# Image-Processing-Systems-Laboratory/DeepInPainting

Measured on AMD Instinct MI355X. Metric: train images/sec at 256x256, batch 8/GPU, 1/2/4/8 MI355X; IPSR layer ms, higher is better.
Workload: dtype f32; 1 GPU; BASELINE config 2: 256x256 synthetic images, 128x128 centre mask (M=256 of N=1024 feature positions), batch 8/GPU, fp32, full IPSR training step; global_batch=8, parallelism=dp1, dropout=True, conv_math=fp32, vgg16=seeded random init (no pretrained weights offline)

## Files before the change

deepinpainting_amd/_lib.py:

```python
import ctypes
import os

_HERE = os.path.dirname(os.path.abspath(__file__))
LIB_PATH = os.path.join(_HERE, "libipsr_hip.so")
ABI_VERSION = 15

_lib = None

c_void_p, c_int, c_float, c_size_t = ctypes.c_void_p, ctypes.c_int, ctypes.c_float, ctypes.c_size_t

SIGNATURES = {
    "ipsr_abi_version": (c_int, []),
    "ipsr_last_error": (ctypes.c_char_p, []),
    "ipsr_feat_mask_workspace_bytes": (c_size_t, [c_int, c_int, c_int]),
    "ipsr_feat_mask": (c_int, [c_void_p, c_int, c_int, c_int, c_float, c_void_p, c_void_p, c_size_t, c_void_p]),
    "ipsr_index_prep": (c_int, [c_void_p, c_int, c_int, c_int, c_int, c_int, c_void_p, c_void_p, c_void_p, c_void_p]),
    "ipsr_patch_normalize": (c_int, [c_void_p, c_int, c_int, c_int, c_void_p, c_void_p, c_void_p]),
    "ipsr_corr_argmax_workspace_bytes": (c_size_t, [c_int, c_int, c_int]),
    "ipsr_corr_argmax": (c_int, [c_void_p, c_void_p, c_int, c_int, c_int, c_void_p, c_void_p, c_void_p,
                                 c_void_p, c_size_t, c_void_p]),
    "ipsr_bwd_index_ints": (c_size_t, [c_int, c_int]),
    "ipsr_forward_workspace_bytes": (c_size_t, [c_int] * 7),
    "ipsr_forward": (c_int, [c_void_p, c_void_p, c_void_p, c_int, c_int, c_int, c_int, c_int, c_int, c_int,
                             c_void_p, c_void_p, c_void_p, c_void_p, c_void_p, c_void_p, c_size_t, c_void_p]),
# ... 65 lines not shown
    "ipsr_l1_pair_loss_workspace_bytes": (c_size_t, [c_int]),
    "ipsr_l1_pair_loss": (c_int, [c_void_p, c_void_p, c_void_p, c_int, c_float, c_void_p, c_void_p, c_void_p, c_void_p, c_size_t, c_void_p]),
    "ipsr_loss_grad_scale": (c_int, [c_void_p, c_void_p, c_void_p, c_int, c_void_p, c_void_p, c_int, c_void_p]),
    "ipsr_profile_enable": (c_int, [c_int]),
    "ipsr_profile_enable_mask": (c_int, [c_int, ctypes.c_uint]),
    "ipsr_profile_read": (c_int, [c_void_p, c_int]),
    "ipsr_profile_read_region": (c_int, [c_int, c_void_p, c_int]),
    "ipsr_profile_read_region_work": (c_int, [c_int, c_void_p, c_void_p, c_int]),
    "ipsr_profile_read_region_work2": (c_int, [c_int, c_void_p, c_void_p, c_void_p, c_int]),
    "ipsr_conv3x3_winograd_mp": (c_int, [c_int, c_void_p, c_void_p, c_void_p, c_int, c_void_p, c_int, c_void_p, c_int, c_int, c_int, c_int, c_int, c_int, c_int,
                                         c_void_p, c_size_t, c_void_p]),
    "ipsr_conv3x3_winograd_wrw_mp": (c_int, [c_int, c_void_p, c_void_p, c_void_p, c_int, c_int, c_int, c_int, c_int, c_int, c_int, c_void_p, c_size_t, c_void_p]),
    "ipsr_conv4x4_winograd_mp": (c_int, [c_int, c_int, c_void_p, c_void_p, c_void_p, c_int, c_int, c_int, c_int, c_int, c_int, c_int, c_void_p, c_size_t, c_void_p]),
    "ipsr_conv4x4s2_winograd_mp": (c_int, [c_int, c_void_p, c_void_p, c_void_p, c_int, c_int, c_int, c_int, c_int, c_int, c_int, c_void_p, c_size_t, c_void_p]),
    "ipsr_conv3x3_bf16_workspace_bytes": (c_size_t, [c_int] * 6),
    "ipsr_conv3x3_bf16x3_workspace_bytes": (c_size_t, [c_int] * 6),
    "ipsr_conv3x3_bf16": (c_int, [c_int, c_void_p, c_void_p, c_void_p, c_int, c_int, c_int, c_int, c_int, c_int, c_void_p, c_size_t, c_void_p]),
    "ipsr_conv3x3_bf16_packed": (c_int, [c_int, c_void_p, c_void_p, c_void_p, c_int, c_int, c_int, c_int, c_int, c_int, c_int, c_void_p, c_size_t, c_void_p]),
    "ipsr_conv4x4s2_bf16_workspace_bytes": (c_size_t, [c_int] * 6),
    "ipsr_conv4x4s2_bf16": (c_int, [c_int, c_void_p, c_void_p, c_void_p, c_int, c_int, c_int, c_int, c_int, c_int, c_void_p, c_size_t, c_void_p]),
    "ipsr_conv4x4s2_bf16_dil_workspace_bytes": (c_size_t, [c_int] * 6),
    "ipsr_conv4x4s2_bf16_dil": (c_int, [c_int, c_void_p, c_void_p, c_void_p, c_int, c_int, c_int, c_int, c_int, c_int, c_void_p, c_size_t, c_void_p]),
    "ipsr_conv4x4s2_bf16x3_workspace_bytes": (c_size_t, [c_int] * 6),
    "ipsr_conv4x4s2_bf16x3": (c_int, [c_int, c_void_p, c_void_p, c_void_p, c_int, c_int, c_int, c_int, c_int, c_void_p, c_size_t, c_void_p]),
    "ipsr_conv4x4s2_bf16_wrw_workspace_bytes": (c_size_t, [c_int] * 5),
    "ipsr_conv4x4s2_bf16_wrw": (c_int, [c_void_p, c_void_p, c_void_p, c_int, c_int, c_int, c_int, c_int, c_void_p, c_size_t, c_void_p]),
    "ipsr_conv4x4s2_bf16x3_wrw_workspace_bytes": (c_size_t, [c_int] * 5),
    "ipsr_conv4x4s2_bf16x3_wrw": (c_int, [c_void_p, c_void_p, c_void_p, c_int, c_int, c_int, c_int, c_int, c_void_p, c_size_t, c_void_p]),
    "ipsr_conv3x3_bf16_wrw_workspace_bytes": (c_size_t, [c_int] * 6),
    "ipsr_conv4x4s2_bf16x3_dil_wrw_workspace_bytes": (c_size_t, [c_int] * 5),
    "ipsr_conv4x4s2_bf16x3_dil_wrw": (c_int, [c_void_p, c_void_p, c_void_p, c_int, c_int, c_int, c_int, c_int, c_void_p, c_size_t, c_void_p]),
    "ipsr_conv3x3_bf16x3_wrw_workspace_bytes": (c_size_t, [c_int] * 6),
    "ipsr_conv3x3_bf16_wrw": (c_int, [c_int, c_void_p, c_void_p, c_void_p, c_int, c_int, c_int, c_int, c_int, c_void_p, c_size_t, c_void_p]),
    "ipsr_wino_gemm_split": (c_int, [c_int, c_int, c_int, c_void_p]),
    "ipsr_debug_force_wino_split": (c_int, [c_int, c_int, c_int]),
    "ipsr_debug_set_option": (c_int, [c_int, c_int]),
}


class IpsrLibraryError(RuntimeError):
    pass


def lib():
    global _lib
    if _lib is not None:
        return _lib
    if not os.path.exists(LIB_PATH):
        raise IpsrLibraryError(
            "libipsr_hip.so not found at %s — build it with `python -c 'import __graft_entry__ as g; g.build()'` "
            "or `make -C deepinpainting_amd/csrc`.  The IPSR layer has no CPU/eager fallback." % LIB_PATH)
    import torch
    h = ctypes.CDLL(LIB_PATH)
    for name, (res, args) in SIGNATURES.items():
        fn = getattr(h, name)
        fn.restype = res
        fn.argtypes = args
    if h.ipsr_abi_version() != ABI_VERSION:
        raise IpsrLibraryError("libipsr_hip.so ABI %d != expected %d — rebuild" % (h.ipsr_abi_version(), ABI_VERSION))
    _lib = h
    return _lib


def check(rc, what):
    if rc == 0:
        return
# ... 5 lines not shown
```

deepinpainting_amd/models/IPSR.py:

```python
import os
from collections import OrderedDict

import torch

from . import networks
from .base_model import BaseModel
from .vgg16 import Vgg16
from .. import dist as ipsr_dist


class IPSR(BaseModel):
    def name(self):
        return 'IPSRModel'

    def initialize(self, opt):
        BaseModel.initialize(self, opt)
        self.opt = opt
        self.isTrain = opt.isTrain
        self.strict_reference = bool(getattr(opt, 'strict_reference', False))
        self.batch_vgg = bool(getattr(opt, 'batch_vgg', False))
        self.batch_disc = bool(getattr(opt, 'batch_disc', True))
        self.amp_bf16 = bool(getattr(opt, 'amp_bf16', False))
        from . import hipconv
        hipconv.set_conv_math(fp32=getattr(opt, 'conv_math', 'fp32'), bf16=getattr(opt, 'conv_math_bf16', 'bf16x3'))
# ... 12 lines not shown
                "seeded-random VGG16 instead.")
        self.vgg = Vgg16(requires_grad=False, weights_path=weights).to(self.device)
        self.vgg.eval()
        if not self.vgg.pretrained and not getattr(opt, 'quiet', False):
            print('WARNING: VGG16 feature extractor is seeded-random (allow_random_vgg) — not the pretrained net the reference uses')

        fs = opt.fineSize
        self.input_A = self.Tensor(opt.batchSize, opt.input_nc, fs, fs)
        self.input_B = self.Tensor(opt.batchSize, opt.output_nc, fs, fs)
        self.input_ref = self.Tensor(opt.batchSize, opt.output_nc, fs, fs)

        self.mask_global = torch.zeros(1, 1, fs, fs, dtype=torch.bool, device=self.device)
        lo, hi = int(fs / 4) + opt.overlap, int(fs / 2) + int(fs / 4) - opt.overlap
        self.mask_global[:, :, lo:hi, lo:hi] = 1
        self.mask_type = opt.mask_type
        self.gMask_opts = {}
        self.use_gpu = len(opt.gpu_ids) > 0

        self.netG, self.Cosis_list, self.Cosis_list2, self.CSA_model = networks.define_G(
            opt.input_nc_g, opt.output_nc, opt.ngf, opt.which_model_netG, opt, self.mask_global, opt.norm,
            opt.use_dropout, opt.init_type, self.gpu_ids, opt.init_gain)
        self.netP, _, _, _ = networks.define_G(
            opt.input_nc, opt.output_nc, opt.ngf, opt.which_model_netP, opt, self.mask_global, opt.norm,
            opt.use_dropout, opt.init_type, self.gpu_ids, opt.init_gain)
        self.CSA_model[0].corr_bf16 = self.amp_bf16 and bool(getattr(opt, 'bf16_corr', True)) and self.device.type == 'cuda'
        if self.isTrain:
            use_sigmoid = opt.gan_type == 'vanilla'
            self.netD = networks.define_D(opt.input_nc, opt.ndf, opt.which_model_netD, opt.n_layers_D, opt.norm,
                                          use_sigmoid, opt.init_type, self.gpu_ids, opt.init_gain)
            self.netF = networks.define_D(opt.input_nc, opt.ndf, opt.which_model_netF, opt.n_layers_D, opt.norm,
                                          use_sigmoid, opt.init_type, self.gpu_ids, opt.init_gain)

        reach = 0 if self.amp_bf16 else int(getattr(opt, 'smallmap_reach', 1024))
        for net in (self.netG, self.netP) + ((self.netD, self.netF) if self.isTrain else ()):
            for mod in net.modules():
                if isinstance(mod, (torch.nn.Conv2d, torch.nn.ConvTranspose2d)):
                    mod.smallmap_reach = reach or None

        if not self.isTrain or opt.continue_train:
            print('Loading pre-trained network!')
            self.load_network(self.netG, 'G', opt.which_epoch)
            self.load_network(self.netP, 'P', opt.which_epoch)
            if self.isTrain:
                self.load_network(self.netD, 'D', opt.which_epoch)
                self.load_network(self.netF, 'F', opt.which_epoch)

        self.criterionGAN = networks.GANLoss(gan_type=opt.gan_type)
        self.criterionL1 = torch.nn.L1Loss()
        self._gt_latent = None
        self._reducer_D = self._reducer_G = None

        if self.isTrain:
            self.old_lr = opt.lr
            fused = bool(getattr(opt, 'fused_adam', True)) and self.device.type == 'cuda'

            def mk(net):
                kw = dict(lr=opt.lr, betas=(opt.beta1, 0.999))
                if fused:
                    try:
                        return torch.optim.Adam(net.parameters(), fused=True, **kw)
                    except (TypeError, RuntimeError):
                        pass
                return torch.optim.Adam(net.parameters(), **kw)
            self.optimizer_G, self.optimizer_P = mk(self.netG), mk(self.netP)
            self.optimizer_D, self.optimizer_F = mk(self.netD), mk(self.netF)
            self.optimizers = [self.optimizer_G, self.optimizer_P, self.optimizer_D, self.optimizer_F]
            self.schedulers = [networks.get_scheduler(o, opt) for o in self.optimizers]

            if torch.distributed.is_available() and torch.distributed.is_initialized() \
                    and torch.distributed.get_world_size() > 1:
# ... 218 lines not shown
```

deepinpainting_amd/models/hipconv.py:

```python
import os
from collections import namedtuple

import torch
import torch.nn as nn
import torch.nn.functional as F

from .. import _lib, ops
from .. import dist as ipsr_dist

_FORCE = None
_MATH = {"fp32": "fp32", "bf16": "bf16x3"}


def set_conv_math(fp32=None, bf16=None):
    from .. import ops as _ops
    for key, val in (("fp32", fp32), ("bf16", bf16)):
        if val is not None:
            if val not in _ops.MATH_CODE or (key == "bf16" and val in _ops.DIRECT_PASSES):
                raise ValueError("conv math must be one of %s" % sorted(k for k in _ops.MATH_CODE if k))
            _MATH[key] = val
    _SEL.clear()


_DIRECT_DILATED = False
# ... 261 lines not shown
    if not (k == 3 and stride == 1 and pad == 1 and dil == 1) or H * W < 4096 or not engine_takes("thin", "data", op, lay, bf16):
        return False
    fwd = op in (ops.CONV_FWD, ops.CONVT_FWD)
    i, o = (Cin, Cout) if fwd else (Cout, Cin)
    if bf16:
        return i == 3
    return o in (3, 6) or i == 3


def _smallmap_op(op):
    return ops.SM_FWD if op in (ops.CONV_FWD, ops.CONVT_BWD_DATA) else ops.SM_DATA


def _smallmap_data_wins(op, lay):
    transposed, B, Cin, H, W, Cout, k, stride, pad, dil = lay
    if _env("IPSR_NO_SMALLMAP", "0") == "1" or k not in (3, 4) or min(Cin, Cout) < 256:
        return False
    g = _smallmap_geometry(lay)
    return g[3] >= 1 and g[4] >= 1 and g[0] * g[3] * g[4] <= int(_env("IPSR_SMALLMAP_MAX_POS", "32")) and engine_takes("smallmap", "data", op, lay, False)


def _smallmap_wrw_wins(lay):
    transposed, B, Cin, H, W, Cout, k, stride, pad, dil = lay
    if k != 4 or stride != 2 or _env("IPSR_NO_SMALLMAP", "0") == "1":
        return False
    g = _smallmap_geometry(lay)
    return g[3] >= 1 and g[4] >= 1 and g[0] * g[3] * g[4] <= 256 and min(Cin, Cout) >= 256 and engine_takes("smallmap", "wrw", None, lay, False)


def _is_k4s1(k, stride, pad, dil):
    return k == 4 and stride == 1 and pad == 1 and dil == 1


def select_wrw(transposed, B, Cin, H, W, Cout, k, stride, pad, dil, bf16=False, reach=None):
    key = (1, _FORCE, transposed, B, Cin, H, W, Cout, k, stride, pad, dil, bf16)
    eng = _SEL.get(key)
    if eng is None:
        eng = _SEL[key] = _select_wrw_any((transposed, B, Cin, H, W, Cout, k, stride, pad, dil), bf16)
    return _reached("wrw", key, eng, None, bf16, reach) if reach else eng


def _select_wrw_any(lay, bf16):
    transposed, B, Cin, H, W, Cout, k, stride, pad, dil = lay
    eng = _select_wrw(lay)
    thin = _mode() == "auto" and _env("IPSR_NO_THIN", "0") != "1" and pad == 1 and dil == 1 and (k, stride) in ((3, 1), (4, 2)) and H * W >= 4096 \
        and engine_takes("thin_mfma", "wrw", None, lay, bf16)
    if not bf16:
        eng = "thin_mfma" if thin and eng == "miopen" else _direct_opt_in("wrw", eng, None, lay)
    elif not (_bf16_wins(eng, Cin, H, W, Cout, True) or _ENGINES[eng].fp32_copies):
        eng = "thin_mfma" if thin else _bf16_direct_wrw(lay)
    return eng if engine_takes(eng, "wrw", None, lay, bf16) else "miopen"


def _bf16_direct_wrw(lay):
    transposed, B, Cin, H, W, Cout, k, stride, pad, dil = lay
    if _env("IPSR_BF16_ENGINES", "") == "none" or _mode() in ("miopen", "winograd", "direct"):
        return "miopen"
    if k == 3 and stride == 1 and pad == 1 and dil == 1 and H * W >= 1024 and engine_takes("bf16d", "wrw", None, lay, True):
        return "bf16d"
    g = _s2_geometry(lay)
    if g is not None and g[3] >= 32 and ((g[0] + 127) // 128) * ((g[1] + 31) // 32) >= 4 and engine_takes("bf16d", "wrw", None, lay, True):
        return "bf16d"
    return "miopen"


def _dil_geometry(lay):
    transposed, B, Cin, H, W, Cout, k, stride, pad, dil = lay
    if transposed or not _is_dilated4(k, stride, pad, dil) or H % 2 or W % 2:
        return None
    return Cout, Cin, H // 2, W // 2


# ... 32 lines not shown
def _select_wrw(lay):
    transposed, B, Cin, H, W, Cout, k, stride, pad, dil = lay
    mode = _mode()
    if mode == "auto" and not transposed and Cout == 1 and Cin >= 64 and engine_takes("one", "wrw", None, lay, False):
        return "one"
    if mode == "auto" and not transposed and _is_dilated4(k, stride, pad, dil) and min(Cin, Cout) >= 128 and 32 <= H <= 128 \
            and H % 2 == 0 and W % 2 == 0:
        return "wino_dil"
    if mode == "auto" and not transposed and _is_k4s1(k, stride, pad, dil) and min(Cin, Cout) >= 128 and 16 <= H <= 128 and W >= 4:
        return "wino_dil"
    if mode == "auto":
        g = _s2_geometry(lay)
        if g is not None and _s2_wins(g):
            return "wino_s2"
    if mode == "auto" and _smallmap_wrw_wins(lay):
        return "smallmap"
    ok = k == 3 and stride == 1 and pad == 1 and dil == 1
    if mode in ("miopen", "direct") or not ok:
        return "miopen"
    if mode == "winograd":
        return "winograd"
    if 256 <= H * W <= 4096 and max(Cin, Cout) >= 256 and min(Cin, Cout) >= 128:
        return "winograd"
    if transposed and Cout == 64 and Cin >= 256 and H * W <= 16384:
        return "winograd"
    return "miopen"


_Engine = namedtuple("_Engine", "data wrw takes bf16_io fp32_copies sink wrw_x_as_dy", defaults=(None, None, None, False, False, False, False))
_K3 = (3, 1, 1, 1)


def engine_takes(eng, kind, op, lay, bf16):
    return eng == "miopen" or bool(_ENGINES[eng].takes(kind, op, lay, bf16))


def _frozen_pack(w, param):
    param = w if param is None else param
    return dict(keep_packed=isinstance(param, nn.Parameter) and not param.requires_grad and not torch.is_grad_enabled(), pack_key=param)


def _fine_coarse(x, dy, lay):
    return ((dy, x) if lay[0] else (x, dy)) + (lay[1],) + _s2_geometry(lay)


def _direct_case(lay, x3):
    if lay[6:] == _K3:
        return "k3", None
    dilated = (x3 or _DIRECT_DILATED_BF16) and _is_dilated4(*lay[6:])
    g = _dil_geometry(lay) if dilated else _s2_geometry(lay)
    return (None if g is None else "dil" if dilated else "s2"), g


def _direct_mode(case, op):
    return _dil_mode(op) if case == "dil" else _s2_mode(op)


def _bf16d_data(op, inp, w, lay, math, out_dtype, param):
    if inp.dtype != torch.bfloat16:
        inp = inp.to(torch.bfloat16)
    case, g = _direct_case(lay, False)
    if case == "k3":
        return ops.conv3x3_bf16(op, inp, w, lay[1:5], lay[5], out_dtype=out_dtype, **_frozen_pack(w, param))
    if case == "dil":
        return ops.conv4x4s2_bf16_dil(_dil_mode(op) & ~ops.S2_DILATED, inp, w, lay[1], *g, out_dtype=out_dtype)
    return ops.conv4x4s2_bf16(_s2_mode(op), inp, w, lay[1], *g, out_dtype=out_dtype)

# ... 90 lines not shown
        lambda op, inp, w, lay, math, out_dtype, param: ops.conv4x4s2_winograd(_s2_mode(op), inp, w, lay[1], *_s2_geometry(lay), math=math, out_dtype=out_dtype),
        lambda x, dy, lay, math, sink: ops.conv4x4s2_winograd(ops.S2_WEIGHT_GRAD, *_fine_coarse(x, dy, lay), out=sink, math=math),
        _wino_s2_takes, bf16_io=True, sink=True, wrw_x_as_dy=True),
    "thin": _Engine(
        lambda op, inp, w, lay, math, out_dtype, param: ops.conv3x3_thin(op, inp, w, lay[1:5], lay[5], out_dtype=out_dtype),
        takes=lambda kind, op, lay, bf16: kind == "data" and lay[6:] == _K3 and ops.thin_supported(op, *lay[2:6])),
    "thin_f2m": _Engine(
        lambda op, inp, w, lay, math, out_dtype, param: ops.conv_thin_f2m_mfma(op, inp, w, lay[1:5], lay[5], lay[6], lay[7], out_dtype=out_dtype),
        takes=lambda kind, op, lay, bf16: kind == "data" and lay[8:] == (1, 1) and ops.thin_f2m_mfma_supported(op, *lay[1:8])),
    "thin_mfma": _Engine(
        None, _thin_mfma_wrw, sink=True,
        takes=lambda kind, op, lay, bf16: kind == "wrw" and lay[8:] == (1, 1) and ops.thin_wrw_mfma_supported(*lay[:8])),
    "smallmap": _Engine(
        lambda op, inp, w, lay, math, out_dtype, param, tiled=False: ops.conv_smallmap(_smallmap_op(op), inp, w, *_smallmap_geometry(lay), tiled=tiled),
        lambda x, dy, lay, math, sink, tiled=False: ops.conv_smallmap(ops.SM_WRW, *((x, dy) if lay[0] else (dy, x)), *_smallmap_geometry(lay), out=sink,
                                                                       tiled=tiled),
        lambda kind, op, lay, bf16, tiled=False: ops.smallmap_supported(_smallmap_op(op) if kind == "data" else ops.SM_WRW, *_smallmap_geometry(lay),
                                                                         tiled=tiled),
        fp32_copies=True, sink=True),
    "direct": _Engine(
        lambda op, inp, w, lay, math, out_dtype, param: ops.conv2d(op, inp, w, lay[1:5], *lay[5:]),
        takes=lambda kind, op, lay, bf16: kind == "data" and ops.conv2d_supported(op, *lay[1:])),
    "one": _Engine(
        lambda op, inp, w, lay, math, out_dtype, param: ops.conv_to_one(inp, w, lay[8]),
        lambda x, dy, lay, math, sink: ops.conv_to_one_wrw(x, dy, lay[6], lay[8], out=sink),
        lambda kind, op, lay, bf16: not lay[0] and lay[5] == 1 and (kind == "wrw" or op == ops.CONV_FWD) and ops.conv_to_one_supported(*lay[1:5], *lay[6:]),
        fp32_copies=True, sink=True),
    "bf16d": _Engine(_bf16d_data, _bf16d_wrw, _bf16d_takes, bf16_io=True, sink=True, wrw_x_as_dy=True),
    "bf16x3d": _Engine(_bf16x3d_data, takes=_bf16x3d_takes),
    "bf16x3w": _Engine(None, _bf16x3w_wrw, _bf16x3w_takes, sink=True),
    "miopen": _Engine(),
}


def _run_data(eng, op, inp, w, lay, math, out_dtype, param=None, tiled=False):
    e = _ENGINES[eng]
    kw = {"tiled": True} if tiled else {}
    if e.fp32_copies:
        return e.data(op, inp.float(), w, lay, math, torch.float32, param, **kw).to(out_dtype)
    return e.data(op, inp, w, lay, math, out_dtype, param, **kw)


def _run_wrw(eng, x, dy, w, lay, math, tiled=False):
    e = _ENGINES[eng]
    sink = ipsr_dist.grad_sink_for(w.data_ptr(), w.shape) if e.sink else None
    if e.fp32_copies:
        x, dy = x.float(), dy.float()
    elif e.wrw_x_as_dy and x.dtype != dy.dtype:
        x = x.to(dy.dtype)
    return e.wrw(x, dy, lay, math, sink, **({"tiled": True} if tiled else {}))


def _miopen_forward(x, w, transposed, stride, pad, dil):
    if x.dtype != w.dtype and not torch.is_autocast_enabled():
        w = w.to(x.dtype)
    return F.conv_transpose2d(x, w, None, stride, pad, 0, 1, dil) if transposed else F.conv2d(x, w, None, stride, pad, dil)


def _miopen_backward(dy, x, w, transposed, stride, pad, dil, which):
    dt = dy.dtype
    out = torch.ops.aten.convolution_backward(dy, x if x.dtype == dt else x.to(dt), w if w.dtype == dt else w.to(dt), None, [stride, stride],
                                              [pad, pad], [dil, dil], transposed, [0, 0], 1, which)
    return out[0], (out[1].to(w.dtype) if out[1] is not None else None)


class _HipConv(torch.autograd.Function):

    @staticmethod
    def forward(ctx, x, w, lay, eng_fwd, math, act, reach=None):
        transposed, B, Cin, H, W, Cout, k, stride, pad, dil = lay
        xc = x.contiguous()
        if eng_fwd == "miopen":
            y = _miopen_forward(xc, w, transposed, stride, pad, dil)
        else:
            fop = ops.CONVT_FWD if transposed else ops.CONV_FWD
            y = _run_data(eng_fwd, fop, xc, w, lay, math, act, tiled=eng_fwd == "smallmap" and _via_reach("data", fop, lay, act == torch.bfloat16, reach))
        ctx.save_for_backward(xc, w)
        ctx.lay, ctx.geom = lay, (transposed, k, stride, pad, dil, Cout)
        ctx.math, ctx.bf16, ctx.reach = math, act == torch.bfloat16, reach
        if _check_hook is not None:
            _check_hook("forward", eng_fwd, ctx.geom, (xc, w), y)
        return y

    @staticmethod
    def backward(ctx, dy):
        x, w = ctx.saved_tensors
        lay, math, bf16, reach = ctx.lay, ctx.math, ctx.bf16, ctx.reach
        transposed, B, Cin, H, W, Cout, k, stride, pad, dil = lay
        dy = dy.contiguous()
        if bf16 and dy.dtype != torch.bfloat16:
            dy = dy.to(torch.bfloat16)
        dx = dw = None
        if ctx.needs_input_grad[0]:
            op = ops.CONVT_BWD_DATA if transposed else ops.CONV_BWD_DATA
            eng = select(op, B, Cin, H, W, Cout, k, stride, pad, dil, bf16, reach=reach)
            if eng == "miopen":
                dx = _miopen_backward(dy, x, w, transposed, stride, pad, dil, [True, False, False])[0]
                if dx.dtype != x.dtype:
                    dx = dx.to(x.dtype)
            else:
                dx = _run_data(eng, op, dy, w, lay, math, x.dtype, tiled=eng == "smallmap" and _via_reach("data", op, lay, bf16, reach))
            if _check_hook is not None:
                _check_hook("input_grad", eng, ctx.geom, (dy, x, w), dx)
        if ctx.needs_input_grad[1]:
            weng = select_wrw(transposed, B, Cin, H, W, Cout, k, stride, pad, dil, bf16, reach=reach)
            if weng == "miopen":
                dw = _miopen_backward(dy, x, w, transposed, stride, pad, dil, [False, True, False])[1]
            else:
                dw = _run_wrw(weng, x, dy, w, lay, math, tiled=weng == "smallmap" and _via_reach("wrw", None, lay, bf16, reach))
            if _check_hook is not None:
                _check_hook("weight_grad", weng, ctx.geom, (dy, x, w), dw)
        return dx, dw, None, None, None, None, None


def _geometry(m):
    ks, st, pd, dl = m.kernel_size, m.stride, m.padding, m.dilation
    if m.groups != 1 or ks[0] != ks[1] or st[0] != st[1] or pd[0] != pd[1] or dl[0] != dl[1] or isinstance(pd, str):
        return None
    if isinstance(m, nn.ConvTranspose2d) and tuple(m.output_padding) != (0, 0):
        return None
    if getattr(m, "padding_mode", "zeros") != "zeros":
        return None
    return ks[0], st[0], pd[0], dl[0]


def _layer_of(m, x, w):
    g = _geometry(m)
    if g is None or not x.is_cuda or x.dim() != 4 or w.dtype != torch.float32 or x.dtype not in (torch.float32, torch.bfloat16):
        return None
    amp = _amp_bf16()
    if not amp and torch.is_autocast_enabled():
        return None
    transposed = isinstance(m, nn.ConvTranspose2d)
    B, Cin, H, W = x.shape
    return (transposed, B, Cin, H, W, w.shape[1] if transposed else w.shape[0]) + g, amp or x.dtype == torch.bfloat16


def conv_math(bf16):
    return _MATH["bf16" if bf16 else "fp32"]


def _engines_of(lay, bf16, dx=True, dw=True, reach=None):
    transposed, B, Cin, H, W, Cout, k, stride, pad, dil = lay
    fop, bop = (ops.CONVT_FWD, ops.CONVT_BWD_DATA) if transposed else (ops.CONV_FWD, ops.CONV_BWD_DATA)
    return (select(fop, B, Cin, H, W, Cout, k, stride, pad, dil, bf16, reach=reach),
            select(bop, B, Cin, H, W, Cout, k, stride, pad, dil, bf16, reach=reach) if dx else "miopen",
            select_wrw(transposed, B, Cin, H, W, Cout, k, stride, pad, dil, bf16, reach=reach) if dw else "miopen")


def any_engine(m, x):
    lb = _layer_of(m, x, m.weight)
    if lb is None:
        return False
    return _engines_of(*lb, reach=getattr(m, "smallmap_reach", None)) != ("miopen",) * 3


def conv_nobias(m, x, weight=None):
    w = m.weight if weight is None else weight
    lb = _layer_of(m, x, w)
    if lb is not None:
        lay, bf16 = lb
        act = torch.bfloat16 if bf16 else torch.float32
        math = _MATH["bf16" if bf16 else "fp32"]
        grad = torch.is_grad_enabled()
        reach = getattr(m, "smallmap_reach", None)
        engs = _engines_of(lay, bf16, grad and x.requires_grad, grad and w.requires_grad, reach)
        if grad and (x.requires_grad or w.requires_grad):
            if engs != ("miopen",) * 3:
                return _HipConv.apply(x, w, lay, engs[0], math, act, reach)
        elif engs[0] != "miopen":
            fop = ops.CONVT_FWD if lay[0] else ops.CONV_FWD
            return _run_data(engs[0], fop, x.contiguous(), w.detach(), lay, math, act, param=w,
                             tiled=engs[0] == "smallmap" and _via_reach("data", fop, lay, bf16, reach))
    if isinstance(m, nn.ConvTranspose2d):
        return F.conv_transpose2d(x, w, None, m.stride, m.padding, m.output_padding, m.groups, m.dilation)
    return F.conv2d(x, w, None, m.stride, m.padding, m.dilation, m.groups)
```

deepinpainting_amd/ops.py:

```python
import contextlib
import threading
import weakref
from collections import namedtuple

import torch

from . import _lib

_ws_cache = {}


def _stream():
    return torch._C._cuda_getCurrentRawStream(torch._C._cuda_getDevice())


def _workspace(nbytes, device):
    key = (device.index, _stream())
    buf = _ws_cache.get(key)
    if buf is None or buf.numel() < nbytes:
        buf = torch.empty(max(int(nbytes), 1 << 20), dtype=torch.uint8, device=device)
        _ws_cache[key] = buf
    return buf


# ... 847 lines not shown
               "ipsr_conv_thin_f2m_mfma")
    return out


def thin_wrw_mfma_supported(transposed, B, Cin, H, W, Cout, k, stride):
    if transposed:
        Kb, Cs, Hb, Wb = Cin, Cout, H, W
    else:
        if H % stride or W % stride:
            return False
        Kb, Cs, Hb, Wb = Cout, Cin, H // stride, W // stride
    return _lib.lib().ipsr_conv_thin_wrw_mfma_workspace_bytes(B, Kb, Cs, Hb, Wb, k, stride) > 0


def conv_thin_wrw_mfma(transposed, x, dy, k, stride, out=None):
    x, _ = _act(x, "x")
    dy, _ = _act(dy, "dy")
    big, small = (x, dy) if transposed else (dy, x)
    if big.dtype == torch.float32 and small.dtype != torch.float32:
        raise TypeError("conv_thin_wrw_mfma: an fp32 wide tensor needs an fp32 narrow one")
    B, Kb, Hb, Wb = big.shape
    Cs = small.shape[1]
    if tuple(small.shape) != (B, Cs, Hb * stride, Wb * stride):
        raise RuntimeError("conv_thin_wrw_mfma: narrow tensor %s does not match wide %s at stride %d" % (tuple(small.shape), tuple(big.shape), stride))
    L = _lib.lib()
    g = _result(out, (Kb, Cs, k, k), torch.float32, x.device, "conv_thin_wrw_mfma")
    ws = _probed_workspace(L, L.ipsr_conv_thin_wrw_mfma_workspace_bytes(B, Kb, Cs, Hb, Wb, k, stride), x.device,
                           "ipsr_conv_thin_wrw_mfma: Kb=%d Cs=%d %dx%d k%d s%d", (Kb, Cs, Hb, Wb, k, stride))
    _lib.check(L.ipsr_conv_thin_wrw_mfma(big.data_ptr(), small.data_ptr(), g.data_ptr(), B, Kb, Cs, Hb, Wb, k, stride, int(big.dtype == torch.bfloat16) | (2 if small.dtype == torch.bfloat16 else 0),
                                         ws.data_ptr(), ws.numel(), _stream()), "ipsr_conv_thin_wrw_mfma")
    return g


SM_DATA, SM_WRW, SM_FWD = 0, 1, 2


SM_TILED = 16


def smallmap_supported(op, B, R, Cq, Ho, Wo, Hf, Wf, k, stride, pad, dil, tiled=False):
    return _lib.lib().ipsr_conv_smallmap_workspace_bytes(op | (SM_TILED if tiled else 0), B, R, Cq, Ho, Wo, Hf, Wf, k, stride, pad, dil) > 0


def conv_smallmap(op, a, b, B, R, Cq, Ho, Wo, Hf, Wf, k, stride, pad, dil, out=None, tiled=False):
    a = _req(a, torch.float32, "operand a")
    b = _req(b, torch.float32, "operand b")
    coarse, fine, wsh = (B, R, Ho, Wo), (B, Cq, Hf, Wf), (R, Cq, k, k)
    want = {SM_DATA: (coarse, wsh, fine), SM_WRW: (coarse, fine, wsh), SM_FWD: (fine, wsh, coarse)}[op]
    if tuple(a.shape) != want[0] or tuple(b.shape) != want[1]:
        raise RuntimeError("conv_smallmap op %d: operands %s / %s do not match %s / %s" % (op, tuple(a.shape), tuple(b.shape), want[0], want[1]))
    out = _result(out, want[2], torch.float32, a.device, "conv_smallmap")
    L = _lib.lib()
    op |= SM_TILED if tiled else 0
    ws = _probed_workspace(L, L.ipsr_conv_smallmap_workspace_bytes(op, B, R, Cq, Ho, Wo, Hf, Wf, k, stride, pad, dil), a.device,
                           "ipsr_conv_smallmap: op %d R=%d Cq=%d %dx%d -> %dx%d k%d s%d p%d d%d", (op, R, Cq, Hf, Wf, Ho, Wo, k, stride, pad, dil))
    _lib.check(L.ipsr_conv_smallmap(op, a.data_ptr(), b.data_ptr(), out.data_ptr(), B, R, Cq, Ho, Wo, Hf, Wf, k, stride, pad, dil,
                                    ws.data_ptr(), ws.numel(), _stream()), "ipsr_conv_smallmap")
    return out


def conv3x3_winograd_wrw(transposed, x, dy, Cout, out=None, math=None):
    x, x_bf = _act(x, "conv input")
    dy, dy_bf = _act(dy, "grad_output")
    if x_bf != dy_bf:
        raise TypeError("conv3x3_winograd_wrw: x and dy must have the same dtype")
    B, Cin, H, W = x.shape
# ... 106 lines not shown
```

deepinpainting_amd/options.py:

```python


class Option(object):
    def __init__(self, **overrides):
        self.batchSize = 1
        self.fineSize = 256
        self.input_nc = 3
        self.input_nc_g = 6
        self.output_nc = 3
        self.ngf = 64
        self.ndf = 64
        self.which_model_netD = 'basic'
        self.which_model_netF = 'feature'
        self.which_model_netG = 'unet_ipsr'
        self.which_model_netP = 'unet_256'
        self.triple_weight = 1
        self.name = 'IPSR_inpainting'
        self.n_layers_D = '3'
        self.gpu_ids = [0]
        self.model = 'ipsr_net'
        self.checkpoints_dir = './checkpoints'
        self.norm = 'instance'
        self.fixed_mask = 1
        self.use_dropout = True
        self.init_type = 'normal'
        self.mask_type = 'random'
        self.lambda_A = 100
        self.threshold = 5 / 16.0
        self.stride = 1
        self.shift_sz = 1
        self.mask_thred = 1
        self.bottleneck = 512
        self.gp_lambda = 10.0
        self.ncritic = 5
        self.constrain = 'MSE'
        self.strength = 1
        self.init_gain = 0.02
        self.cosis = 1
        self.gan_type = 'lsgan'
        self.gan_weight = 0.2
        self.overlap = 4
        self.skip = 0
        self.display_freq = 1000
        self.print_freq = 50
        self.save_latest_freq = 5000
        self.save_epoch_freq = 1
        self.continue_train = False
        self.epoch_count = 1
        self.phase = 'train'
        self.which_epoch = ''
        self.niter = 20
        self.niter_decay = 100
        self.beta1 = 0.5
        self.lr = 0.0002
        self.lr_policy = 'lambda'
        self.lr_decay_iters = 50
        self.isTrain = True
        self.smallmap_reach = 1024
        for k, v in overrides.items():
            setattr(self, k, v)
```

include/ipsr_hip.h:

```cpp
#ifndef IPSR_HIP_H
#define IPSR_HIP_H

#include <stddef.h>
#include <stdint.h>

#ifdef __cplusplus
extern "C" {
#endif

#define IPSR_OK                 0
#define IPSR_ERR_INVALID       -1
#define IPSR_ERR_UNSUPPORTED   -2
#define IPSR_ERR_WORKSPACE     -3
#define IPSR_ERR_LAUNCH        -4

int ipsr_abi_version(void);
const char* ipsr_last_error(void);

size_t ipsr_feat_mask_workspace_bytes(int H, int W, int layers);
int ipsr_feat_mask(const uint8_t* mask, int H, int W, int layers, float threshold,
                   uint8_t* feat, void* ws, size_t ws_bytes, void* stream);

int ipsr_index_prep(const uint8_t* feat, int h, int w, int patch, int stride, int mask_thred,
                    int32_t* flag , int32_t* mask_point_idx , int32_t* count ,
// ... 151 lines not shown
                             int math, int io, void* ws, size_t ws_bytes, void* stream);
int ipsr_conv4x4s2_winograd_mp(int mode, const void* a, const void* b, void* out, int B, int Kc, int Cf, int nh, int nw,
                               int math, int io, void* ws, size_t ws_bytes, void* stream);

size_t ipsr_conv3x3_bf16_workspace_bytes(int op, int B, int Cin, int H, int W, int Cout);
size_t ipsr_conv3x3_bf16x3_workspace_bytes(int op, int B, int Cin, int H, int W, int Cout);
int ipsr_conv3x3_bf16(int op, const void* in, const float* weight, void* out, int B, int Cin, int H, int W, int Cout, int io,
                      void* ws, size_t ws_bytes, void* stream);
int ipsr_conv3x3_bf16_packed(int op, const void* in, const float* weight, void* out, int B, int Cin, int H, int W, int Cout, int io,
                             int pack_valid, void* ws, size_t ws_bytes, void* stream);
size_t ipsr_conv4x4s2_bf16_workspace_bytes(int mode, int B, int Kc, int Cf, int nh, int nw);
int ipsr_conv4x4s2_bf16(int mode, const void* in, const float* weight, void* out, int B, int Kc, int Cf, int nh, int nw, int out_bf16,
                        void* ws, size_t ws_bytes, void* stream);
size_t ipsr_conv4x4s2_bf16_dil_workspace_bytes(int mode, int B, int Kc, int Cf, int nh, int nw);
int ipsr_conv4x4s2_bf16_dil(int mode, const void* in, const float* weight, void* out, int B, int Kc, int Cf, int nh, int nw, int out_bf16,
                            void* ws, size_t ws_bytes, void* stream);
size_t ipsr_conv4x4s2_bf16x3_workspace_bytes(int mode, int B, int Kc, int Cf, int nh, int nw);
int ipsr_conv4x4s2_bf16x3(int mode, const float* in, const float* weight, float* out, int B, int Kc, int Cf, int nh, int nw,
                          void* ws, size_t ws_bytes, void* stream);
size_t ipsr_conv4x4s2_bf16_wrw_workspace_bytes(int B, int Kc, int Cf, int nh, int nw);
int ipsr_conv4x4s2_bf16_wrw(const void* fine, const void* coarse, float* dw, int B, int Kc, int Cf, int nh, int nw,
                            void* ws, size_t ws_bytes, void* stream);
size_t ipsr_conv4x4s2_bf16x3_wrw_workspace_bytes(int B, int Kc, int Cf, int nh, int nw);
int ipsr_conv4x4s2_bf16x3_wrw(const float* fine, const float* coarse, float* dw, int B, int Kc, int Cf, int nh, int nw,
                              void* ws, size_t ws_bytes, void* stream);
size_t ipsr_conv4x4s2_bf16x3_dil_wrw_workspace_bytes(int B, int Kc, int Cf, int nh, int nw);
int ipsr_conv4x4s2_bf16x3_dil_wrw(const float* fine, const float* coarse, float* dw, int B, int Kc, int Cf, int nh, int nw,
                                  void* ws, size_t ws_bytes, void* stream);
size_t ipsr_conv3x3_bf16_wrw_workspace_bytes(int transposed, int B, int Cin, int H, int W, int Cout);
size_t ipsr_conv3x3_bf16x3_wrw_workspace_bytes(int transposed, int B, int Cin, int H, int W, int Cout);
int ipsr_conv3x3_bf16_wrw(int form, const void* x, const void* dy, float* dw, int B, int Cin, int H, int W, int Cout,
                          void* ws, size_t ws_bytes, void* stream);

int ipsr_wino_gemm_split(int rows, int cols, int reduction, int* out5 );
int ipsr_debug_force_wino_split(int nsplit, int xi_split, int nsplit_tail);
int ipsr_debug_set_option(int key, int value);

#ifdef __cplusplus
}
#endif
#endif
```

Before: 364.4 images/sec.

## Add fp32 MFMA weight-gradient kernel for three conv shapes replacing MIOpen

Adds a HIP kernel that computes conv weight gradients in fp32 using 32x32x2 f32 MFMA. It stages the big map in double-buffered LDS and the small map in a row ring buffer, writes per-run partial slabs, and sums them with a separate reduce kernel. It is enabled by default for three specific layer geometries that previously fell back to MIOpen, selected through an allowlist. It adds workspace memory and an extra reduce pass, and only covers channel counts that are multiples of 64.

```diff
diff --git a/deepinpainting_amd/_lib.py b/deepinpainting_amd/_lib.py
--- a/deepinpainting_amd/_lib.py
+++ b/deepinpainting_amd/_lib.py
@@ -121,6 +121,8 @@
     "ipsr_conv4x4s2_bf16x3_dil_wrw": (c_int, [c_void_p, c_void_p, c_void_p, c_int, c_int, c_int, c_int, c_int, c_void_p, c_size_t, c_void_p]),
     "ipsr_conv3x3_bf16x3_wrw_workspace_bytes": (c_size_t, [c_int] * 6),
     "ipsr_conv3x3_bf16_wrw": (c_int, [c_int, c_void_p, c_void_p, c_void_p, c_int, c_int, c_int, c_int, c_int, c_void_p, c_size_t, c_void_p]),
+    "ipsr_conv_wrw_f32_workspace_bytes": (c_size_t, [c_int] * 6),
+    "ipsr_conv_wrw_f32": (c_int, [c_int, c_void_p, c_void_p, c_void_p, c_int, c_int, c_int, c_int, c_int, c_void_p, c_size_t, c_void_p]),
     "ipsr_wino_gemm_split": (c_int, [c_int, c_int, c_int, c_void_p]),
     "ipsr_debug_force_wino_split": (c_int, [c_int, c_int, c_int]),
     "ipsr_debug_set_option": (c_int, [c_int, c_int]),
diff --git a/deepinpainting_amd/csrc/conv_f32_wrw.hip b/deepinpainting_amd/csrc/conv_f32_wrw.hip
--- /dev/null
+++ b/deepinpainting_amd/csrc/conv_f32_wrw.hip
@@ -0,0 +1,263 @@
+#include "ipsr_common.h"
+
+namespace ipsr {
+namespace {
+
+typedef float wrw_f32x16 __attribute__((ext_vector_type(16)));
+
+enum { WRW_K3 = 0, WRW_S2 = 1, WRW_DIL = 2 };
+constexpr int WRW_CUS = 256;
+
+template <int K, int ST>
+struct WrwTile {
+    static constexpr int XS = ST == 1 ? 64 : 32;
+    static constexpr int LDA = XS + 1;
+    static constexpr int SW = (XS - 1) * ST + K;
+    static constexpr int LDS_ROW = SW | 1;
+    static constexpr int RING = K + ST;
+    static constexpr int THREADS = 256 * K;
+    static constexpr int NB = (64 * XS + THREADS - 1) / THREADS;
+    static constexpr int NS = (64 * SW + THREADS - 1) / THREADS;
+    static constexpr size_t LDS_BYTES = (size_t)(2 * 64 * LDA + RING * 64 * LDS_ROW) * sizeof(float);
+};
+
+struct WrwArgs {
+    const float* big;
+    const float* small;
+    float* slabs;
+    int A, C, Hb, Wb;
+    int Hp, Wp;
+    size_t splane;
+    int srow, scol, soff;
+    int pad;
+    int nxseg, rows_per_run, chunks;
+};
+
+template <int K, int ST>
+__global__ void __launch_bounds__(256 * K) wrw_f32_kernel(const WrwArgs g)
+{
+    using T = WrwTile<K, ST>;
+    extern __shared__ __attribute__((aligned(16))) float wrw_lds[];
+    float* const bigbuf = wrw_lds;
+    float* const ring = wrw_lds + 2 * 64 * T::LDA;
+
+    const int tid = threadIdx.x, lane = tid & 63, wave = tid >> 6;
+    const int n = lane & 31, h = lane >> 5;
+    const int quad = wave & 3, r = wave >> 2;
+    const int m0 = (quad & 1) * 32, c0l = (quad >> 1) * 32;
+
+    const int run = blockIdx.x;
+    const int chunk = run % g.chunks, col = run / g.chunks;
+    const int xs = col % g.nxseg, b = col / g.nxseg;
+    const int a0 = blockIdx.y * 64, c0 = blockIdx.z * 64;
+    const int x0 = xs * T::XS;
+    const int y0 = chunk * g.rows_per_run, y1 = min(g.Hb, y0 + g.rows_per_run);
+
+    const float* const bigp = g.big + ((size_t)b * g.A + a0) * g.Hb * g.Wb;
+    const float* const smallp = g.small + ((size_t)b * g.C + c0) * g.splane;
+    const size_t bplane = (size_t)g.Hb * g.Wb;
+    const int pc0 = x0 * ST - g.pad;
+
+    float rb[T::NB], rs[ST][T::NS];
+    auto load_big = [&](int y) {
+#pragma unroll
+        for (int i = 0; i < T::NB; ++i) {
+            const int e = min(tid + i * T::THREADS, 64 * T::XS - 1);
+            const int ch = e / T::XS, px = e - ch * T::XS;
+            const int x = x0 + px;
+            const float v = bigp[(size_t)ch * bplane + (size_t)y * g.Wb + min(x, g.Wb - 1)];
+            rb[i] = x < g.Wb ? v : 0.0f;
+        }
+    };
+    auto store_big = [&](int buf) {
+#pragma unroll
+        for (int i = 0; i < T::NB; ++i) {
+            const int e = tid + i * T::THREADS;
+            const int ch = e / T::XS, px = e - ch * T::XS;
+            if (e < 64 * T::XS) bigbuf[(buf * 64 + ch) * T::LDA + px] = rb[i];
+        }
+    };
+    auto load_small = [&](int prow, int j) {
+        const bool rowok = (unsigned)prow < (unsigned)g.Hp;
+        const size_t rbase = (size_t)min(max(prow, 0), g.Hp - 1) * g.srow + g.soff;
+#pragma unroll
+        for (int i = 0; i < T::NS; ++i) {
+            const int e = min(tid + i * T::THREADS, 64 * T::SW - 1);
+            const int ch = e / T::SW, q = e - ch * T::SW;
+            const int pc = pc0 + q;
+            const float v = smallp[(size_t)ch * g.splane + rbase + (size_t)min(max(pc, 0), g.Wp - 1) * g.scol];
+            rs[j][i] = (rowok && (unsigned)pc < (unsigned)g.Wp) ? v : 0.0f;
+        }
+    };
+    auto store_small = [&](int prow, int j) {
+        const int slot = (prow + g.pad) % T::RING;
+#pragma unroll
+        for (int i = 0; i < T::NS; ++i) {
+            const int e = tid + i * T::THREADS;
+            const int ch = e / T::SW, q = e - ch * T::SW;
+            if (e < 64 * T::SW) ring[(slot * 64 + ch) * T::LDS_ROW + q] = rs[j][i];
+        }
+    };
+
+    wrw_f32x16 acc[K];
+#pragma unroll
+    for (int s = 0; s < K; ++s)
+#pragma unroll
+        for (int e = 0; e < 16; ++e) acc[s][e] = 0.0f;
+
+    for (int j = 0; j < K; ++j) {
+        load_small(y0 * ST - g.pad + j, 0);
+        store_small(y0 * ST - g.pad + j, 0);
+    }
+    load_big(y0);
+    store_big(0);
+    __syncthreads();
+
+    for (int y = y0; y < y1; ++y) {
+        const int cur = (y - y0) & 1;
+        const bool more = y + 1 < y1;
+        if (more) {
+            load_big(y + 1);
+#pragma unroll
+            for (int j = 0; j < ST; ++j) load_small(y * ST - g.pad + K + j, j);
+        }
+        {
+            const int slot = (y * ST + r) % T::RING;
+            const float* const ap = bigbuf + (cur * 64 + m0 + n) * T::LDA + h;
+            const float* const sp = ring + (slot * 64 + c0l + n) * T::LDS_ROW + h * ST;
+#pragma unroll 4
+            for (int p = 0; p < T::XS; p += 2) {
+                const float a = ap[p];
+#pragma unroll
+                for (int s = 0; s < K; ++s) acc[s] = __builtin_amdgcn_mfma_f32_32x32x2f32(a, sp[p * ST + s], acc[s], 0, 0, 0);
+            }
+        }
+        if (more) {
+            store_big(cur ^ 1);
+#pragma unroll
+            for (int j = 0; j < ST; ++j) store_small(y * ST - g.pad + K + j, j);
+        }
+        __syncthreads();
+    }
+
+    const size_t slab = ((size_t)blockIdx.y * gridDim.z + blockIdx.z) * gridDim.x + run;
+    float* const out = g.slabs + slab * (size_t)(K * K * 64 * 64);
+#pragma unroll
+    for (int s = 0; s < K; ++s)
+#pragma unroll
+        for (int e = 0; e < 16; ++e) {
+            const int row = m0 + (e & 3) + 8 * (e >> 2) + 4 * h;
+            out[((r * K + s) * 64 + row) * 64 + c0l + n] = acc[s][e];
+        }
+}
+
+__global__ void __launch_bounds__(256) wrw_f32_reduce_kernel(const float* __restrict__ slabs, float* __restrict__ dW, int C, int taps, int ctiles, int nruns)
+{
+    __shared__ float part[4][64];
+    const int cl = threadIdx.x & 63, grp = threadIdx.x >> 6;
+    const int al = blockIdx.x & 63, tap = (blockIdx.x >> 6) % taps, tile = (blockIdx.x >> 6) / taps;
+    const size_t sstride = (size_t)taps * 64 * 64;
+    const float* p = slabs + (size_t)tile * nruns * sstride + ((size_t)tap * 64 + al) * 64 + cl;
+    float s0 = 0.0f, s1 = 0.0f, s2 = 0.0f, s3 = 0.0f;
+    int i = grp;
+    for (; i + 12 < nruns; i += 16) {
+        s0 += p[(size_t)i * sstride]; s1 += p[(size_t)(i + 4) * sstride]; s2 += p[(size_t)(i + 8) * sstride]; s3 += p[(size_t)(i + 12) * sstride];
+    }
+    for (; i < nruns; i += 4) s0 += p[(size_t)i * sstride];
+    part[grp][cl] = (s0 + s1) + (s2 + s3);
+    __syncthreads();
+    if (grp == 0) {
+        const int a = (tile / ctiles) * 64 + al, c = (tile % ctiles) * 64 + cl;
+        dW[((size_t)a * C + c) * taps + tap] = ((part[0][cl] + part[1][cl]) + part[2][cl]) + part[3][cl];
+    }
+}
+
+struct WrwPlan {
+    int K, ST, pad, xs;
+    int atiles, ctiles, nxseg, rows_per_run, chunks, nruns;
+};
+
+bool wrw_f32_plan(int geom, int B, int A, int C, int Hb, int Wb, WrwPlan* p)
+{
+    if (geom < WRW_K3 || geom > WRW_DIL || B < 1 || A < 64 || C < 64 || A % 64 || C % 64 || Hb < 1 || Wb < 1) return false;
+    p->K = geom == WRW_K3 ? 3 : 4;
+    p->ST = geom == WRW_S2 ? 2 : 1;
+    p->pad = geom == WRW_DIL ? 2 : 1;
+    p->xs = p->ST == 1 ? 64 : 32;
+    p->atiles = A / 64;
+    p->ctiles = C / 64;
+    p->nxseg = cdiv(Wb, p->xs);
+    const long cols = (long)B * p->nxseg, tiles = (long)p->atiles * p->ctiles;
+    if (p->atiles > 65535 || p->ctiles > 65535 || tiles > (1L << 20) || cols * Hb > (1L << 30) || Hb > (1 << 29) || Wb > (1 << 29)) return false;
+    long chunks = WRW_CUS / (tiles * cols);
+    chunks = chunks < 1 ? 1 : chunks > Hb ? Hb : chunks;
+    int rows = cdiv(Hb, (int)chunks);
+    if (debug_option(7) > 0) rows = debug_option(7) < Hb ? debug_option(7) : Hb;
+    p->rows_per_run = rows;
+    p->chunks = cdiv(Hb, rows);
+    p->nruns = (int)(cols * p->chunks);
+    return true;
+}
+
+template <int K, int ST>
+int wrw_f32_launch(const WrwArgs& g, const WrwPlan& p, hipStream_t st)
+{
+    using T = WrwTile<K, ST>;
+    static_assert(T::LDS_BYTES <= 160 * 1024, "the staging buffers exceed the LDS");
+    static bool raised = false;
+    if (!raised) {
+        if (hipFuncSetAttribute(reinterpret_cast<const void*>(&wrw_f32_kernel<K, ST>), hipFuncAttributeMaxDynamicSharedMemorySize, (int)T::LDS_BYTES) != hipSuccess)
+            return fail(IPSR_ERR_LAUNCH, "ipsr_conv_wrw_f32: cannot raise the dynamic LDS limit to %zu bytes", T::LDS_BYTES);
+        raised = true;
+    }
+    wrw_f32_kernel<K, ST><<<dim3(p.nruns, p.atiles, p.ctiles), T::THREADS, T::LDS_BYTES, st>>>(g);
+    return check_launch("wrw_f32_kernel");
+}
+
+}
+}
+
+using namespace ipsr;
+
+extern "C" {
+
+size_t ipsr_conv_wrw_f32_workspace_bytes(int geom, int B, int Kb, int Cs, int Hb, int Wb)
+{
+    WrwPlan p;
+    if (!wrw_f32_plan(geom, B, Kb, Cs, Hb, Wb, &p)) return 0;
+    return align_up((size_t)p.atiles * p.ctiles * p.nruns * p.K * p.K * 64 * 64 * sizeof(float), 256);
+}
+
+int ipsr_conv_wrw_f32(int geom, const float* big, const float* small, float* dw, int B, int Kb, int Cs, int Hb, int Wb,
+                      void* ws, size_t ws_bytes, void* stream)
+{
+    if (!big || !small || !dw || !ws) return fail(IPSR_ERR_INVALID, "ipsr_conv_wrw_f32: null pointer");
+    if ((reinterpret_cast<uintptr_t>(big) | reinterpret_cast<uintptr_t>(small) | reinterpret_cast<uintptr_t>(dw) | reinterpret_cast<uintptr_t>(ws)) & 3u)
+        return fail(IPSR_ERR_INVALID, "ipsr_conv_wrw_f32: operands, result and workspace must be 4-byte aligned");
+    WrwPlan p;
+    if (!wrw_f32_plan(geom, B, Kb, Cs, Hb, Wb, &p))
+        return fail(IPSR_ERR_UNSUPPORTED, "ipsr_conv_wrw_f32: geometry %d, B=%d Kb=%d Cs=%d %dx%d is not implemented (k3 s1 p1 / k4 s2 p1 / k4 s2 p3 d2, "
+                    "channel counts multiples of 64)", geom, B, Kb, Cs, Hb, Wb);
+    const size_t need = ipsr_conv_wrw_f32_workspace_bytes(geom, B, Kb, Cs, Hb, Wb);
+    if (ws_bytes < need) return fail(IPSR_ERR_WORKSPACE, "ipsr_conv_wrw_f32: workspace %zu < %zu", ws_bytes, need);
+    hipStream_t st = static_cast<hipStream_t>(stream);
+    WrwArgs g;
+    g.big = big; g.small = small; g.slabs = static_cast<float*>(ws);
+    g.A = Kb; g.C = Cs; g.Hb = Hb; g.Wb = Wb;
+    const int Hs = geom == WRW_K3 ? Hb : 2 * Hb, Ws = geom == WRW_K3 ? Wb : 2 * Wb;
+    g.splane = (size_t)Hs * Ws;
+    if (geom == WRW_DIL) { g.Hp = Hb; g.Wp = Wb; g.srow = 2 * Ws; g.scol = 2; g.soff = Ws + 1; }
+    else { g.Hp = Hs; g.Wp = Ws; g.srow = Ws; g.scol = 1; g.soff = 0; }
+    g.pad = p.pad;
+    g.nxseg = p.nxseg; g.rows_per_run = p.rows_per_run; g.chunks = p.chunks;
+    int rc;
+    if (geom == WRW_K3) rc = wrw_f32_launch<3, 1>(g, p, st);
+    else if (geom == WRW_S2) rc = wrw_f32_launch<4, 2>(g, p, st);
+    else rc = wrw_f32_launch<4, 1>(g, p, st);
+    if (rc) return rc;
+    const int taps = p.K * p.K;
+    wrw_f32_reduce_kernel<<<p.atiles * p.ctiles * taps * 64, 256, 0, st>>>(g.slabs, dw, Cs, taps, p.ctiles, p.nruns);
+    return check_launch("wrw_f32_reduce_kernel");
+}
+
+}
diff --git a/deepinpainting_amd/models/IPSR.py b/deepinpainting_amd/models/IPSR.py
--- a/deepinpainting_amd/models/IPSR.py
+++ b/deepinpainting_amd/models/IPSR.py
@@ -68,10 +68,12 @@
                                           use_sigmoid, opt.init_type, self.gpu_ids, opt.init_gain)
 
         reach = 0 if self.amp_bf16 else int(getattr(opt, 'smallmap_reach', 1024))
+        wrw_f32 = not self.amp_bf16 and bool(int(getattr(opt, 'wrw_f32', 1)))
         for net in (self.netG, self.netP) + ((self.netD, self.netF) if self.isTrain else ()):
             for mod in net.modules():
                 if isinstance(mod, (torch.nn.Conv2d, torch.nn.ConvTranspose2d)):
                     mod.smallmap_reach = reach or None
+                    mod.wrw_f32 = wrw_f32 or None
 
         if not self.isTrain or opt.continue_train:
             print('Loading pre-trained network!')
diff --git a/deepinpainting_amd/models/hipconv.py b/deepinpainting_amd/models/hipconv.py
--- a/deepinpainting_amd/models/hipconv.py
+++ b/deepinpainting_amd/models/hipconv.py
@@ -317,12 +317,33 @@
     return k == 4 and stride == 1 and pad == 1 and dil == 1
 
 
-def select_wrw(transposed, B, Cin, H, W, Cout, k, stride, pad, dil, bf16=False, reach=None):
+def select_wrw(transposed, B, Cin, H, W, Cout, k, stride, pad, dil, bf16=False, reach=None, wrw_f32=None):
     key = (1, _FORCE, transposed, B, Cin, H, W, Cout, k, stride, pad, dil, bf16)
     eng = _SEL.get(key)
     if eng is None:
         eng = _SEL[key] = _select_wrw_any((transposed, B, Cin, H, W, Cout, k, stride, pad, dil), bf16)
-    return _reached("wrw", key, eng, None, bf16, reach) if reach else eng
+    if reach:
+        eng = _reached("wrw", key, eng, None, bf16, reach)
+    return _wrw_f32_moved(key, eng, bf16) if wrw_f32 else eng
+
+
+_WRW_F32_ROWS = frozenset({
+    (False, 64, 256, 256, 64, 4, 2, 3, 2),
+    (False, 64, 128, 128, 128, 3, 1, 1, 1),
+    (True, 64, 128, 128, 64, 4, 2, 1, 1),
+})
+
+
+def _wrw_f32_moved(key, eng, bf16):
+    if eng != "miopen" or bf16:
+        return eng
+    wkey = key + ("wrw_f32",)
+    hit = _SEL.get(wkey)
+    if hit is None:
+        lay = key[2:-1]
+        ok = _mode() == "auto" and (lay[0],) + lay[2:] in _WRW_F32_ROWS and bool(_WRW_F32.takes("wrw", None, lay, False))
+        hit = _SEL[wkey] = "wrw_f32" if ok else eng
+    return hit
 
 
 def _select_wrw_any(lay, bf16):
@@ -421,7 +442,7 @@
 
 
 def engine_takes(eng, kind, op, lay, bf16):
-    return eng == "miopen" or bool(_ENGINES[eng].takes(kind, op, lay, bf16))
+    return eng == "miopen" or bool(_record(eng).takes(kind, op, lay, bf16))
 
 
 def _frozen_pack(w, param):
@@ -578,6 +599,14 @@
     "miopen": _Engine(),
 }
 
+_WRW_F32 = _Engine(
+    None, lambda x, dy, lay, math, sink: ops.conv_wrw_f32(lay[0], x, dy, *lay[6:], out=sink),
+    lambda kind, op, lay, bf16: kind == "wrw" and not bf16 and ops.conv_wrw_f32_supported(*lay), sink=True)
+
+
+def _record(eng):
+    return _WRW_F32 if eng == "wrw_f32" else _ENGINES[eng]
+
 
 def _run_data(eng, op, inp, w, lay, math, out_dtype, param=None, tiled=False):
     e = _ENGINES[eng]
@@ -588,7 +617,7 @@
 
 
 def _run_wrw(eng, x, dy, w, lay, math, tiled=False):
-    e = _ENGINES[eng]
+    e = _record(eng)
     sink = ipsr_dist.grad_sink_for(w.data_ptr(), w.shape) if e.sink else None
     if e.fp32_copies:
         x, dy = x.float(), dy.float()
@@ -613,7 +642,7 @@
 class _HipConv(torch.autograd.Function):
 
     @staticmethod
-    def forward(ctx, x, w, lay, eng_fwd, math, act, reach=None):
+    def forward(ctx, x, w, lay, eng_fwd, math, act, reach=None, wrw_f32=None):
         transposed, B, Cin, H, W, Cout, k, stride, pad, dil = lay
         xc = x.contiguous()
         if eng_fwd == "miopen":
@@ -623,7 +652,7 @@
             y = _run_data(eng_fwd, fop, xc, w, lay, math, act, tiled=eng_fwd == "smallmap" and _via_reach("data", fop, lay, act == torch.bfloat16, reach))
         ctx.save_for_backward(xc, w)
         ctx.lay, ctx.geom = lay, (transposed, k, stride, pad, dil, Cout)
-        ctx.math, ctx.bf16, ctx.reach = math, act == torch.bfloat16, reach
+        ctx.math, ctx.bf16, ctx.reach, ctx.wrw_f32 = math, act == torch.bfloat16, reach, wrw_f32
         if _check_hook is not None:
             _check_hook("forward", eng_fwd, ctx.geom, (xc, w), y)
         return y
@@ -649,14 +678,14 @@
             if _check_hook is not None:
                 _check_hook("input_grad", eng, ctx.geom, (dy, x, w), dx)
         if ctx.needs_input_grad[1]:
-            weng = select_wrw(transposed, B, Cin, H, W, Cout, k, stride, pad, dil, bf16, reach=reach)
+            weng = select_wrw(transposed, B, Cin, H, W, Cout, k, stride, pad, dil, bf16, reach=reach, wrw_f32=ctx.wrw_f32)
             if weng == "miopen":
                 dw = _miopen_backward(dy, x, w, transposed, stride, pad, dil, [False, True, False])[1]
             else:
                 dw = _run_wrw(weng, x, dy, w, lay, math, tiled=weng == "smallmap" and _via_reach("wrw", None, lay, bf16, reach))
             if _check_hook is not None:
                 _check_hook("weight_grad", weng, ctx.geom, (dy, x, w), dw)
-        return dx, dw, None, None, None, None, None
+        return dx, dw, None, None, None, None, None, None
 
 
 def _geometry(m):
@@ -686,19 +715,19 @@
     return _MATH["bf16" if bf16 else "fp32"]
 
 
-def _engines_of(lay, bf16, dx=True, dw=True, reach=None):
+def _engines_of(lay, bf16, dx=True, dw=True, reach=None, wrw_f32=None):
     transposed, B, Cin, H, W, Cout, k, stride, pad, dil = lay
     fop, bop = (ops.CONVT_FWD, ops.CONVT_BWD_DATA) if transposed else (ops.CONV_FWD, ops.CONV_BWD_DATA)
     return (select(fop, B, Cin, H, W, Cout, k, stride, pad, dil, bf16, reach=reach),
             select(bop, B, Cin, H, W, Cout, k, stride, pad, dil, bf16, reach=reach) if dx else "miopen",
-            select_wrw(transposed, B, Cin, H, W, Cout, k, stride, pad, dil, bf16, reach=reach) if dw else "miopen")
+            select_wrw(transposed, B, Cin, H, W, Cout, k, stride, pad, dil, bf16, reach=reach, wrw_f32=wrw_f32) if dw else "miopen")
 
 
 def any_engine(m, x):
     lb = _layer_of(m, x, m.weight)
     if lb is None:
         return False
-    return _engines_of(*lb, reach=getattr(m, "smallmap_reach", None)) != ("miopen",) * 3
+    return _engines_of(*lb, reach=getattr(m, "smallmap_reach", None), wrw_f32=getattr(m, "wrw_f32", None)) != ("miopen",) * 3
 
 
 def conv_nobias(m, x, weight=None):
@@ -710,10 +739,11 @@
         math = _MATH["bf16" if bf16 else "fp32"]
         grad = torch.is_grad_enabled()
         reach = getattr(m, "smallmap_reach", None)
-        engs = _engines_of(lay, bf16, grad and x.requires_grad, grad and w.requires_grad, reach)
+        wrw_f32 = getattr(m, "wrw_f32", None)
+        engs = _engines_of(lay, bf16, grad and x.requires_grad, grad and w.requires_grad, reach, wrw_f32)
         if grad and (x.requires_grad or w.requires_grad):
             if engs != ("miopen",) * 3:
-                return _HipConv.apply(x, w, lay, engs[0], math, act, reach)
+                return _HipConv.apply(x, w, lay, engs[0], math, act, reach, wrw_f32)
         elif engs[0] != "miopen":
             fop = ops.CONVT_FWD if lay[0] else ops.CONV_FWD
             return _run_data(engs[0], fop, x.contiguous(), w.detach(), lay, math, act, param=w,
diff --git a/deepinpainting_amd/ops.py b/deepinpainting_amd/ops.py
--- a/deepinpainting_amd/ops.py
+++ b/deepinpainting_amd/ops.py
@@ -903,6 +903,47 @@
     return g
 
 
+WRW_F32_GEOMS = {(3, 1, 1, 1): 0, (4, 2, 1, 1): 1, (4, 2, 3, 2): 2}
+
+
+def _wrw_f32_args(transposed, B, Cin, H, W, Cout, k, stride, pad, dil):
+    geom = WRW_F32_GEOMS.get((k, stride, pad, dil))
+    if geom is None or (transposed and geom == 2):
+        return None
+    if transposed:
+        return geom, B, Cin, Cout, H, W
+    if H % stride or W % stride:
+        return None
+    return geom, B, Cout, Cin, H // stride, W // stride
+
+
+def conv_wrw_f32_supported(transposed, B, Cin, H, W, Cout, k, stride, pad, dil):
+    a = _wrw_f32_args(transposed, B, Cin, H, W, Cout, k, stride, pad, dil)
+    return a is not None and _lib.lib().ipsr_conv_wrw_f32_workspace_bytes(*a) > 0
+
+
+def conv_wrw_f32(transposed, x, dy, k, stride, pad, dil, out=None):
+    x = _req(x, torch.float32, "x")
+    dy = _req(dy, torch.float32, "dy")
+    B, Cin, H, W = x.shape
+    Cout = dy.shape[1]
+    a = _wrw_f32_args(transposed, B, Cin, H, W, Cout, k, stride, pad, dil)
+    if a is None:
+        raise NotImplementedError("conv_wrw_f32: k%d s%d p%d d%d %s on a %dx%d map is not implemented" % (
+            k, stride, pad, dil, "ConvTranspose2d" if transposed else "Conv2d", H, W))
+    geom, _, Kb, Cs, Hb, Wb = a
+    big, small = (x, dy) if transposed else (dy, x)
+    hs, ws_ = (Hb, Wb) if geom == 0 else (2 * Hb, 2 * Wb)
+    if tuple(big.shape) != (B, Kb, Hb, Wb) or tuple(small.shape) != (B, Cs, hs, ws_):
+        raise RuntimeError("conv_wrw_f32: x %s / dy %s do not match k%d s%d p%d d%d" % (tuple(x.shape), tuple(dy.shape), k, stride, pad, dil))
+    L = _lib.lib()
+    dw = _result(out, (Kb, Cs, k, k), torch.float32, x.device, "conv_wrw_f32")
+    ws = _probed_workspace(L, L.ipsr_conv_wrw_f32_workspace_bytes(*a), x.device, "ipsr_conv_wrw_f32: geom %d B=%d Kb=%d Cs=%d %dx%d", a)
+    _lib.check(L.ipsr_conv_wrw_f32(geom, big.data_ptr(), small.data_ptr(), dw.data_ptr(), B, Kb, Cs, Hb, Wb, ws.data_ptr(), ws.numel(), _stream()),
+               "ipsr_conv_wrw_f32")
+    return dw
+
+
 SM_DATA, SM_WRW, SM_FWD = 0, 1, 2
 
 
diff --git a/deepinpainting_amd/options.py b/deepinpainting_amd/options.py
--- a/deepinpainting_amd/options.py
+++ b/deepinpainting_amd/options.py
@@ -56,5 +56,6 @@
         self.lr_decay_iters = 50
         self.isTrain = True
         self.smallmap_reach = 1024
+        self.wrw_f32 = 1
         for k, v in overrides.items():
             setattr(self, k, v)
diff --git a/include/ipsr_hip.h b/include/ipsr_hip.h
--- a/include/ipsr_hip.h
+++ b/include/ipsr_hip.h
@@ -207,6 +207,10 @@
 int ipsr_conv3x3_bf16_wrw(int form, const void* x, const void* dy, float* dw, int B, int Cin, int H, int W, int Cout,
                           void* ws, size_t ws_bytes, void* stream);
 
+size_t ipsr_conv_wrw_f32_workspace_bytes(int geom, int B, int Kb, int Cs, int Hb, int Wb);
+int ipsr_conv_wrw_f32(int geom, const float* big, const float* small, float* dw, int B, int Kb, int Cs, int Hb, int Wb,
+                      void* ws, size_t ws_bytes, void* stream);
+
 int ipsr_wino_gemm_split(int rows, int cols, int reduction, int* out5 );
 int ipsr_debug_force_wino_split(int nsplit, int xi_split, int nsplit_tail);
 int ipsr_debug_set_option(int key, int value);
```

Result: no change. 365.7 images/sec, median of 4 (+0.4%).
